# stevebottos/owl-vit-object-detection

Measured on AMD Instinct MI355X. Metric: train images/sec, OWL-ViT-B/16 768x768, higher is better.
Workload: dtype bf16; 1 GPU; owlvit-base-patch16 bf16, batch=32/GPU, 768x768, full train step (matcher+loss+backward+AdamW); global_batch=32, parallelism=dp1, encoder_streams=2, weights=init, optimizer_schedule=in-line, windows=1

## Files before the change

### include/owl_hip.h

```cpp
#ifndef OWL_HIP_H
#define OWL_HIP_H
#include <stdint.h>

#ifdef __cplusplus
extern "C" {
#endif

#define OWL_ABI_VERSION 8
const char* owl_last_error(void);
int owl_abi_version(void);

int owl_gemm_nt_bf16(void* stream, int epi, const void* A, int64_t lda, int64_t a_rows, const void* W, int64_t ldw, int64_t w_rows, const float* bias, void* out, int64_t ldo, const float* resid, void* aux, int64_t ld_aux, int64_t M, int64_t N, int64_t K, float alpha, int splits, int64_t Tp, int tile);
#define OWL_GEMM_KERNEL_SP128 0
#define OWL_GEMM_KERNEL_SP256 1
#define OWL_GEMM_KERNEL_PP2 2
#define OWL_GEMM_KERNEL_PPH 3
int owl_gemm_nt_plan(int epi, int64_t M, int64_t N, int64_t K, int64_t a_rows, int has_aux, int64_t Tp, int splits, int tile, int* kernels, int64_t* rows);
int owl_gemm_effective_splits(int64_t K, int splits);
int owl_gemm_slab_workspace_bytes(int64_t M, int64_t ldo, int64_t K, int splits, int64_t* bytes);
int owl_slab_reduce(void* stream, const float* slabs, float* out, int64_t n, int64_t slab_stride, int nsplit, int accumulate);

int owl_patch_embed_scratch_bytes(int64_t B, int64_t S, int64_t ps, int64_t D, int tile, int64_t* bytes);
int owl_patch_embed_bf16(void* stream, const void* image_bf16, const void* w_pe, const float* pos, float* x_out, void* scratch, int64_t B, int64_t S, int64_t ps, int64_t D, int64_t Tp, int tile);
int owl_cls_rows(void* stream, float* x, const float* cls, const float* pos, int64_t B, int64_t Tp, int64_t D);
// ... 41 lines not shown
int owl_preprocess_color_workspace_bytes(int64_t n_tiles, int64_t out_h, int64_t out_w, int64_t* bytes);
int owl_preprocess_u8_tiles_color(void* stream, const void* desc, const float* color, int64_t n_tiles, int64_t max_rows, unsigned char* tmp, void* workspace, int64_t workspace_bytes, const float* lut, void* out, int out_bf16, int64_t n_out, int64_t out_h, int64_t out_w);
int owl_normalize_u8(void* stream, const unsigned char* src, int src_chw, const float* lut, void* out, int out_bf16, int64_t n_images, int64_t H, int64_t W);

int owl_text_embed(void* stream, const int64_t* ids, const float* tok_emb, const float* pos_emb, float* x, int64_t N, int64_t S, int64_t W, int64_t vocab);
int owl_causal_attention_small(void* stream, const void* qkv_bf16, void* out_bf16, int64_t N, int64_t S, int64_t heads, float scale);
int owl_text_pool_project(void* stream, const float* x, const int64_t* ids, const float* gamma, const float* beta, const float* wproj, float* out, int64_t N, int64_t S, int64_t W, int64_t Pdim, float eps);

int owl_gemm_tn_slab_bf16(void* stream, const void* dY, int64_t ldy, const void* X, int64_t ldx, const void* zero_row, float* slab, int64_t M, int64_t N, int64_t K, int splits, int* splits_used, int variant, float* bias_slab);
int owl_colsum_bf16(void* stream, const void* in_bf16, int64_t ld, float* colsum, int64_t R, int64_t C, float* partials, int64_t partials_floats);
int owl_gemm_tn_slab_workspace_bytes(int64_t M, int64_t N, int64_t K, int splits, int64_t* bytes);

int owl_box_pairwise(void* stream, const float* boxes1, const float* boxes2, float* out3, int64_t N, int64_t M);

int owl_rowreduce_workspace_bytes(int64_t groups, int64_t rows_per_group, int64_t C, int64_t* bytes);
int owl_layernorm_bwd(void* stream, const void* dy, int dy_bf16, const float* x, const float* stats, const float* gamma, const float* dres, float* dx, float* dgamma, float* dbeta, int64_t rows, int64_t D, void* dx_bf16, float* partials, int64_t partials_floats, float* dx_colsum);
int owl_merge_ln_bwd(void* stream, const float* dfeats, const float* x, const float* cls_ln, const float* stats1, const float* stats2, const float* g1, const float* b1, const float* g2, float* dx, float* dcls_ws, float* dg1, float* db1, float* dg2, float* db2, int64_t B, int64_t P, int64_t Tp, int64_t D, float* partials, int64_t partials_floats, void* dx_bf16, float* dx_colsum);
int owl_class_sims_bwd(void* stream, const float* dsims, const float* sims, const unsigned char* argmax, const float* inv_norm, const float* e, const float* qhat32, void* de_bf16, void* g_bf16, void* e_bf16, int64_t rows, int64_t Dt, int64_t C);
int owl_query_normalize_bwd(void* stream, const float* dqhat, const float* queries, float* dqueries, int64_t nq, int64_t Dt);
int owl_class_sims_wide_bwd(void* stream, const float* dsims, const float* sims, const unsigned char* argmax, const float* inv_norm, const float* e, const float* qhat_wide, void* de_bf16, void* g_bf16, void* e_bf16, int64_t rows, int64_t Dt, int64_t C, int64_t Qp);
int owl_query_normalize_wide_bwd(void* stream, const float* dqhat_wide, const float* queries, float* dqueries, int64_t nq, int64_t Dt);
int owl_box_final_bwd_blocks(int64_t rows);
int owl_box_final_bwd(void* stream, const float* dboxes, const float* sig, const void* h1_bf16, const void* u1_bf16, const float* w2, void* du1_bf16, float* partials, float* dw2_db2, int64_t rows, int64_t D, float* du1_colsum);
int owl_transpose_colsum_bf16(void* stream, const void* in, int64_t ld_in, void* out_t, int64_t ld_out, float* colsum, int64_t R, int64_t C, float* partials, int64_t partials_floats);
int owl_colsum_f32(void* stream, const float* in, float* colsum, int64_t R, int64_t C, float* partials, int64_t partials_floats);
int owl_embed_bwd(void* stream, const float* dx, float* dpos, float* dcls, void* dE_bf16, int64_t B, int64_t T, int64_t Tp, int64_t D);
int owl_im2row_bf16(void* stream, const void* image_bf16, void* out_bf16, int64_t ld_out, int64_t B, int64_t S, int64_t ps);
int owl_slab_reduce_rows(void* stream, const float* slabs, float* out, int64_t rows, int64_t cols, int64_t ld_slab, int64_t slab_stride, int nsplit, int accumulate);

int owl_adamw_step(void* stream, float* p, const float* g, float* m, float* v, void* p_bf16, int64_t n, float lr, float beta1, float beta2, float eps, float weight_decay, int64_t step, float grad_scale);

int owl_grad_norm_workspace_bytes(int64_t n, int64_t* bytes);
int owl_grad_sumsq(void* stream, const float* g, int64_t n, void* workspace);
int owl_adamw_step_grouped(void* stream, float* p, const float* g, float* m, float* v, void* p_bf16, int64_t n, float lr, float beta1, float beta2, float eps, float weight_decay, int64_t step, float grad_scale, const int64_t* seg_end, const float* seg_lr, const float* seg_wd, int nseg, float max_norm, const void* workspace, float* norm_out);

int owl_ema_update(void* stream, float* ema, const float* p, int64_t n, float d, float w);
int owl_adamw_step_ema(void* stream, float* p, const float* g, float* m, float* v, void* p_bf16, int64_t n, float lr, float beta1, float beta2, float eps, float weight_decay, int64_t step, float grad_scale, const int64_t* seg_end, const float* seg_lr, const float* seg_wd, int nseg, float max_norm, const void* workspace, float* norm_out, float* ema, float d, float w);

int owl_prefix_emit(void* stream, const float* xs, const void* delta1_bf16, const void* delta2_bf16, int64_t n, int64_t block_elems, const int64_t* dst_addr, const int64_t* slot_addr);
int owl_prefix_gather(void* stream, int64_t n, int64_t block_elems, const int64_t* src_addr, const int64_t* dst_addr);

int owl_image_query_workspace_bytes(int64_t N, int64_t P, int64_t Dt, int64_t* nbytes);
int owl_image_query_select(void* stream, const float* e, const float* boxes, const float* qbox, int64_t N, int64_t P, int64_t Dt, void* workspace, int64_t workspace_bytes, int* best, float* query, int* info, float* v_out, double* mean_out, double* sim_out);
int owl_query_bank_fill(void* stream, const float* query, const int* row_ptr, const int* members, float* bank, int64_t N, int64_t nq, int64_t Dt);

int owl_class_logits_fwd(void* stream, const float* e, const float* queries, const void* feats_bf16, const float* w_shift, const float* b_shift, const float* w_scale, const float* b_scale, const unsigned char* mask, float* rowstats, float* logits, float* scores, int64_t B, int64_t P, int64_t Q, int64_t nbanks, int64_t nmasks, int64_t Dt, int64_t D);
// ... 23 lines not shown
```

### owl-vit-object-detection_amd/autograd.py

```python
from collections import namedtuple

import torch

from . import _lib, ops


DW_ITEMS = 256
TN_SMALL_N = True
FOLD_BIAS_COLSUM = True


def _grads_attached(model) -> bool:
    for n, off in model.flat_offsets.items():
        g = model._byname[n].grad
        if g is None or g.data_ptr() != model.flat_grad.data_ptr() + 4 * off:
            return False
    return True


def _attach_grads(model):
    if _grads_attached(model):
        return
    keep = {}
    for n in model.flat_offsets:
# ... 85 lines not shown
            if head["event"] is not None:
                main.wait_event(head["event"])
        else:
            backward_impl(model, B, d_boxes, None, None, logit_head=head)
        hg = (None,) * ctx.n_head
        if dhead is not None:
            hg = (dhead[:D], dhead[2 * D:2 * D + 1], dhead[D:2 * D], dhead[2 * D + 1:])
        return (None, None, dq, None) + (None,) * nflat + hg


def _bws(model, B):
    key = ("bwd", B)
    if key in model._ws:
        return model._ws[key]
    cfg, dev = model.cfg, model.device_
    D, I, Tp, P, Dt, H = cfg.hidden, cfg.mlp, cfg.tokens_padded, cfg.patches, cfg.text_dim, cfg.heads
    M, Mh = B * Tp, B * P
    Mp, Mhp = ops.pad_rows(M), ops.pad_rows(Mh)
    bf, f32 = torch.bfloat16, torch.float32
    z = ops.zeros_rows
    Qg = _routed_cols(model)
    sz = _dw_sizes(cfg, Qg, model._train_emb)
    ws = dict(
        de=z(Mh, Dt, bf, dev), dqhat=torch.zeros(Qg, Dt, device=dev), du1=z(Mh, D, bf, dev), du0=z(Mh, D, bf, dev),
        g32=z(Mh, Qg, bf, dev), e_bf=z(Mh, Dt, bf, dev),
        box_part=torch.zeros(_lib.load().owl_box_final_bwd_blocks(Mh), 5 * D + 4, device=dev),
        slab=torch.zeros(sz.slab, device=dev),
        sink=torch.zeros(4 * D + 8, device=dev),
        bslab=torch.zeros(256 * max(3 * D, I, Dt), device=dev), bslab2=torch.zeros(256 * max(D, Dt), device=dev),
        dfeats=z(Mh, D, f32, dev), dcls=torch.zeros(B, D, device=dev),
        dx=z(M, D, f32, dev), dxb=z(M, D, bf, dev), du=z(M, I, bf, dev), dh=z(M, D, bf, dev), dxm=z(M, D, f32, dev),
        datt=z(M, D, bf, dev), dqkv=z(M, 3 * D, bf, dev),
        dvec=torch.zeros(B, H, Tp, device=dev),
        part=ops.rowreduce_workspace(B, Tp, max(3 * D, I, Dt), dev),
        part2=ops.rowreduce_workspace(B, Tp, max(3 * D, I, Dt), dev),
        dxb2=z(M, D, bf, dev),
        tA=torch.zeros(sz.tok_rows, Mp, dtype=bf, device=dev) if sz.tok_rows else None,
        tB=torch.zeros(sz.tok_rows, Mp, dtype=bf, device=dev) if sz.tok_rows else None,
        tAh=torch.zeros(sz.tAh_rows, Mhp, dtype=bf, device=dev),
        tBh=torch.zeros(sz.tBh_rows, Mhp, dtype=bf, device=dev),
        wT=torch.zeros(max(3 * D, I) * max(D, I), dtype=bf, device=dev),
        slab2=torch.zeros(sz.slab2, device=dev),
        wT2=torch.zeros(Dt * D, dtype=bf, device=dev),
        tn_all=sz.tn_all,
    )
    ws["dw_main"] = dict(slab=ws["slab"], part=ws["part"], bslab=ws["bslab"], tA=ws["tAh"], tB=ws["tBh"], tn_all=sz.tn_all)
    ws["dw_class"] = dict(slab=ws["slab2"], part=ws["part2"], bslab=ws["bslab2"], tA=ws["tAh"], tB=ws["tBh"], tn_all=sz.tn_all)
    ws["dw_enc"] = dict(slab=ws["slab"], part=ws["part2"], bslab=ws["bslab"], tA=ws["tA"], tB=ws["tB"], tn_all=sz.tn_all)
    model._ws[key] = ws
    return ws


def _split_k(n_rows_out, n_cols_out, k):
    t = 256 if (n_rows_out >= 512 and n_cols_out >= 256) else 128
    tiles = ((n_rows_out + t - 1) // t) * ((n_cols_out + t - 1) // t)
    slots = 256 if t == 256 else 512
    return max(1, min(k // 64, slots // tiles))


def _qkv_grads(model, i):
    D, pre = model.cfg.hidden, f"backbone.encoder.layers.{i}.self_attn.q_proj."
    o, ob = model.flat_offsets[pre + "weight"], model.flat_offsets[pre + "bias"]
    return model.flat_grad[o: o + 3 * D * D].view(3 * D, D), model.flat_grad[ob: ob + 3 * D]


def _routed_cols(model):
    return ops.wide_qp(model.cfg.n_classes) if model.wide_head else 32


DwPlan = namedtuple("DwPlan", "tn splits n_in_pad slab_elems")
DwSizes = namedtuple("DwSizes", "tn_all slab slab2 tok_rows tAh_rows tBh_rows")


def _dw_plan(n_out, n_in, *, bias=False, tn_all=False, rows=None):
    if n_in % 256 == 0 and (n_out % 256 == 0 or (TN_SMALL_N and n_out % 8 == 0 and n_out <= 64 and tn_all and not bias)):
# ... 46 lines not shown
    if scratch is None:
        plan, ld, dev = _dw_plan(D, K), ops.pad_rows(rows), dE.device
        scratch = dict(slab=torch.zeros(plan.slab_elems, device=dev),
                       tA=None if plan.tn else torch.zeros(D, ld, dtype=torch.bfloat16, device=dev), tB=None if plan.tn else torch.zeros(K, ld, dtype=torch.bfloat16, device=dev))
    weight_grad(dE, patches, grad_w, D, K, rows, scratch, accumulate=accumulate)


def backward_impl(model, B, d_boxes, d_sims, sims, logit_head=None):
    cfg = model.cfg
    D, I, H, Tp, T, P, Dt, C = cfg.hidden, cfg.mlp, cfg.heads, cfg.tokens_padded, cfg.tokens, cfg.patches, cfg.text_dim, cfg.n_classes
    M, Mh = B * Tp, B * P
    ws, bw = model._workspace(B), _bws(model, B)
    P_ = model._byname
    model._wait_params()
    model._grad_clean = False
    _attach_grads(model)
    G = lambda n: P_[n].grad
    tv = model._tview
    units, tls, floor, low = model._units, model._tl_set, model.backward_floor, model._chain_low
    t_q, t_cls, t_box = "queries" in units, "class_predictor.dense0" in units, "box_head" in units
    below_heads = floor != "heads"
    below_enc = floor in ("pre_layernorm", "embeddings")
    LP = lambda i: f"backbone.encoder.layers.{i}."
    d_boxes = d_boxes.contiguous().float()
    if logit_head is None:
        d_sims = d_sims.contiguous().float()
    else:
        d_logits = logit_head["dlogits"].contiguous().float()

    pre_wt = model._wt if (getattr(model, "pretranspose", False) and model._wt_event is not None) else None
    if pre_wt is not None:
        torch.cuda.current_stream().wait_event(model._wt_event)

    def wT(name, rows, cols, buf=bw["wT"]):
        if name not in model.flat_offsets:
            return model._fz[name + ".T"]
        if pre_wt is not None:
            return pre_wt[name]
        out = buf[: rows * cols].view(cols, rows)
        ops.transpose_bf16(tv(name), out, rows, cols)
        return out

    S, J, fork = model._bwd_streams()
    main0 = torch.cuda.current_stream()
    hs = S(1) if (model.head_streams and model.encoder_streams > 1 and len(model._encoder_chunks(B)) > 1 and bw["tn_all"]) else main0
    ev_h = model._dw_events
# ... 21 lines not shown
                                     workspace=bw[key], **more)
                if t_cls:
                    weight_grad(bw["de"], ws["feats"], G("class_predictor.dense0.weight"), Dt, D, Mh, cdw, G("class_predictor.dense0.bias"))
                if below_heads:
                    ops.gemm(ops.EPI_ACC_F32, bw["de"], wT("class_predictor.dense0.weight", Dt, D, buf=cw), bw["dfeats"], M=Mh, N=D, K=Dt)
        elif t_q or t_cls or below_heads:
            if model.wide_head:
                Qp = bw["g32"].shape[1]
                ops.class_sims_wide_bwd(d_sims, sims, ws["argmax"], ws["inv_norm"], ws["e"], ws["qhat"], bw["de"], bw["g32"], bw["e_bf"], Mh, Dt, C)
                if t_q:
                    weight_grad(bw["g32"], bw["e_bf"], bw["dqhat"], Qp, Dt, Mh, cdw, accumulate=0)
                    ops.query_normalize_wide_bwd(bw["dqhat"], P_["queries"], G("queries"), cfg.queries, Dt)
            else:
                ops.class_sims_bwd(d_sims, sims, ws["argmax"], ws["inv_norm"], ws["e"], ws["qhat"], bw["de"], bw["g32"], bw["e_bf"], Mh, Dt, C)
                if t_q:
                    weight_grad(bw["g32"], bw["e_bf"], bw["dqhat"], 32, Dt, Mh, cdw, accumulate=0)
                    _lib.call("owl_query_normalize_bwd", ops.stream(), bw["dqhat"], P_["queries"], G("queries"), cfg.queries, Dt)
            if t_cls:
                weight_grad(bw["de"], ws["feats"], G("class_predictor.dense0.weight"), Dt, D, Mh, cdw, G("class_predictor.dense0.bias"))
            if below_heads:
                ops.gemm(ops.EPI_F32, bw["de"], wT("class_predictor.dense0.weight", Dt, D, buf=cw), bw["dfeats"], M=Mh, N=D, K=Dt)
        if hs is not main0:
            ev_h[1].record(hs)
    w0T = None
    if t_box or below_heads:
        if t_box:
            gw2, gb2 = G("box_head.dense2.weight"), G("box_head.dense2.bias")
            assert gb2.data_ptr() == gw2.data_ptr() + 4 * gw2.numel(), "dense2 weight/bias grads must be adjacent in the flat bucket"
        else:
            gw2 = bw["sink"]
        ops.box_final_bwd(d_boxes, ws["sig"], ws["hb1"], ws["ub1"], P_["box_head.dense2.weight"], bw["du1"], bw["box_part"], gw2, Mh, D,
                          du1_colsum=G("box_head.dense1.bias") if t_box else None)
        if t_box:
            weight_grad(bw["du1"], ws["hb0"], G("box_head.dense1.weight"), D, D, Mh, bw["dw_main"])
        ops.gemm(ops.EPI_DGELU_BF16, bw["du1"], wT("box_head.dense1.weight", D, D), bw["du0"], aux=ws["ub0"], M=Mh, N=D, K=D)
        if t_box:
            weight_grad(bw["du0"], ws["feats"], G("box_head.dense0.weight"), D, D, Mh, bw["dw_main"], G("box_head.dense0.bias"))
        if below_heads:
            w0T = wT("box_head.dense0.weight", D, D)
    if hs is not main0:
        main0.wait_event(ev_h[1])
    if logit_head is not None and logit_head.get("event") is not None:
        logit_head["event"].record(main0)
    if not below_heads:
        return
    ops.gemm(ops.EPI_ACC_F32, bw["du0"], w0T, bw["dfeats"], M=Mh, N=D, K=D)
    sink = bw["sink"]
    t_pl, t_ppl = "backbone.post_layernorm" in units, "post_post_layernorm" in units
    last = cfg.layers - 1
    ops.merge_ln_bwd(bw["dfeats"], ws["x_fin"], ws["cls_ln"], ws["st_post"], ws["st_pp"], P_["backbone.post_layernorm.weight"],
                     P_["backbone.post_layernorm.bias"], P_["post_post_layernorm.weight"], bw["dx"], bw["dcls"],
                     G("backbone.post_layernorm.weight") if t_pl else sink[:D], G("backbone.post_layernorm.bias") if t_pl else sink[D:2 * D],
                     G("post_post_layernorm.weight") if t_ppl else sink[2 * D:3 * D], G("post_post_layernorm.bias") if t_ppl else sink[3 * D:4 * D],
                     B, P, Tp, D, partials=bw["part"], dx_bf16=bw["dxb"],
                     dx_colsum=G(LP(last) + "mlp.fc2.bias") if last in tls else None)
    if low is None:
        return
    scale = cfg.head_dim ** -0.5

    def dx_only(layers):
        chunks = model._encoder_chunks(B)
        main = torch.cuda.current_stream()
        streams = [main] + [S(c) for c in range(1, len(chunks))]
        if len(chunks) > 1:
            fork.record(main)
            for s_ in streams[1:]:
                s_.wait_event(fork)
        for i in layers:
            Ls, fz = model._layer_ws(B, i), model._fz
# ... 101 lines not shown
```

### owl-vit-object-detection_amd/losses.py

```python
import torch
import torch.nn as nn

from . import _lib, ops
from .matcher import HungarianMatcher, PackedTargets, box_iou, generalized_box_iou
from .matcher import OpenVocabMatcher, _mask_u8, pack_open_vocab_targets


class _PushPullFn(torch.autograd.Function):
    @staticmethod
    def forward(ctx, pred_sims, pred_boxes, crit, tg):
        B, P, C = pred_sims.shape
        dev = pred_sims.device
        sims = pred_sims.detach().contiguous().float()
        boxes = pred_boxes.detach().contiguous().float()
        tc, pred_idx, tgt_idx, _ = crit.matcher.match_packed(sims, boxes, tg)
        s = ops.stream()
        _lib.call("owl_spread_labels", s, boxes, tc, B, P, crit.background_label, 0.85)
        need = pred_sims.requires_grad or pred_boxes.requires_grad
        per_image = torch.empty(B, 4, device=dev)
        losses = torch.empty(4, device=dev)
        dsims = torch.empty(B, P, C, device=dev) if need else None
        dl1 = torch.empty(B, P, 4, device=dev) if need else None
        dgiou = torch.empty(B, P, 4, device=dev) if need else None
        _lib.call("owl_push_pull_loss", s, sims, boxes, tc, crit.scales, tg.boxes, pred_idx, tgt_idx, tg.counts, per_image,
                  losses, dsims, dl1, dgiou, B, P, C, tg.Nmax, crit.background_label)
        ctx.saved = (tc, dsims, dl1, dgiou, B, P, C, crit.background_label)
        crit.last = dict(target_classes=tc, pred_idx=pred_idx, tgt_idx=tgt_idx, per_image=per_image, sizes=tg.sizes)
        return losses[0], losses[1], losses[2], losses[3]

    @staticmethod
    def backward(ctx, g0, g1, g2, g3):
        tc, dsims, dl1, dgiou, B, P, C, bg = ctx.saved
        dev = tc.device
        g = torch.stack([g0, g1, g2, g3]).to(device=dev, dtype=torch.float32)
        out_sims = torch.empty(B, P, C, device=dev)
        out_boxes = torch.empty(B, P, 4, device=dev)
        _lib.call("owl_push_pull_loss_bwd", ops.stream(), g, tc, dsims, dl1, dgiou, out_sims, out_boxes, B, P, C, bg)
        return out_sims, out_boxes, None, None


class PushPullLoss(nn.Module):
    def __init__(self, n_classes, scales):
        super().__init__()
        self.matcher = HungarianMatcher(n_classes)
        self.scales = None if scales is None else torch.as_tensor(scales, dtype=torch.float32)
        self.background_label = n_classes
        self.last = None

    def pack(self, target_classes, target_boxes, device):
        if isinstance(target_classes, PackedTargets):
            return target_classes
        labels = list(target_classes) if not torch.is_tensor(target_classes) else list(target_classes.unbind(0))
        boxes = list(target_boxes) if not torch.is_tensor(target_boxes) else list(target_boxes.unbind(0))
        return PackedTargets(labels, boxes, device, self.background_label)

    def forward(self, predicted_classes, target_classes, predicted_boxes, target_boxes=None):
        dev = predicted_classes.device
        if self.scales is not None and self.scales.device != dev:
            self.scales = self.scales.to(dev)
        tg = self.pack(target_classes, target_boxes, dev)
        if len(tg.sizes) != predicted_classes.shape[0]:
# ... 2 lines not shown
        return {"loss_ce": ce, "loss_bg": bg, "loss_bbox": l1, "loss_giou": giou}


class _OpenVocabFn(torch.autograd.Function):
    @staticmethod
    def forward(ctx, logits, pred_boxes, crit, tg, mask_u8, nmasks, num_boxes):
        B, P, Q = logits.shape
        dev = logits.device
        lg = logits.detach().contiguous().float()
        boxes = pred_boxes.detach().contiguous().float()
        tc, pred_idx, tgt_idx, _ = crit.matcher.match_packed(lg, boxes, tg, mask_u8, nmasks)
        s = ops.stream()
        need = logits.requires_grad or pred_boxes.requires_grad
        nbytes = torch.zeros(1, dtype=torch.int64)
        _lib.call("owl_focal_loss_workspace_bytes", B, P, Q, nbytes)
        ws = torch.empty(int(nbytes.item()) // 8, dtype=torch.float64, device=dev)
        losses = torch.empty(3, device=dev)
        dl1 = torch.empty(B, P, 4, device=dev) if need else None
        dgiou = torch.empty(B, P, 4, device=dev) if need else None
        _lib.call("owl_focal_loss_fwd", s, lg, mask_u8, tc, ws, ws.numel() * 8, B, P, Q, nmasks, float(crit.alpha))
        _lib.call("owl_box_pair_loss", s, boxes, mask_u8, tg.labels, tg.boxes, pred_idx, tgt_idx, tg.counts, ws, ws.numel() * 8, dl1, dgiou, B, P, Q, nmasks, tg.Nmax)
        _lib.call("owl_open_vocab_loss_reduce", s, ws, ws.numel() * 8, losses, B, P, Q, float(num_boxes))
        ctx.saved = (lg, mask_u8, nmasks, tc, dl1, dgiou, float(crit.alpha), float(num_boxes))
        crit.last = dict(target_classes=tc, pred_idx=pred_idx, tgt_idx=tgt_idx, sizes=tg.sizes, num_boxes=float(num_boxes))
        return losses[0], losses[1], losses[2]

    @staticmethod
    def backward(ctx, g0, g1, g2):
        lg, mask_u8, nmasks, tc, dl1, dgiou, alpha, num_boxes = ctx.saved
        B, P, Q = lg.shape
        dev = lg.device
        g = torch.stack([g0, g1, g2]).to(device=dev, dtype=torch.float32)
        dlogits = torch.empty(B, P, Q, device=dev)
        dboxes = torch.empty(B, P, 4, device=dev)
        s = ops.stream()
        _lib.call("owl_focal_loss_bwd", s, g, lg, mask_u8, tc, dlogits, B, P, Q, nmasks, alpha, num_boxes)
        _lib.call("owl_box_pair_loss_bwd", s, g, dl1, dgiou, dboxes, B, P, num_boxes)
        return dlogits, dboxes, None, None, None, None, None


class OpenVocabLoss(nn.Module):

    def __init__(self, alpha=0.25, class_cost=1, bbox_cost=5, giou_cost=2, gamma=2, box_format="xyxy"):
        super().__init__()
        if gamma != 2:
            raise ValueError("OpenVocabLoss: gamma is 2 (the kernels square the modulating factor); other values are not built")
        if box_format not in ("xyxy", "cxcywh"):
            raise ValueError(f"box_format must be 'xyxy' or 'cxcywh', got {box_format!r}")
        self.matcher = OpenVocabMatcher(class_cost, bbox_cost, giou_cost)
        self.alpha = float(alpha)
        self.box_format = box_format
        self.last = None

    def forward(self, logits, pred_boxes, targets, query_mask=None, num_boxes=None):
        if logits.dim() != 3 or pred_boxes.shape != logits.shape[:2] + (4,):
            raise ValueError("logits must be [B, P, Q] and pred_boxes [B, P, 4]")
        B, P, Q = logits.shape
        tg = pack_open_vocab_targets(targets, logits.device, Q, query_mask, self.box_format)
        if len(tg.sizes) != B:
            raise ValueError("batch size mismatch between predictions and targets")
        if tg.Nmax > P:
# ... 9 lines not shown
```

### owl-vit-object-detection_amd/models.py

```python
import math
from collections import OrderedDict

import numpy as np
import torch
import torch.nn as nn

from . import _lib, ops, weights as W
from .config import OwlConfig, check_image_size, get_config, table_grid
from .postprocess import PostProcess
from .prefix_cache import PrefixCache, _id_list


def box_bias_table(grid: int) -> torch.Tensor:
    coords = torch.arange(1, grid + 1, dtype=torch.float32)
    xx, yy = torch.meshgrid(coords, coords, indexing="xy")
    bc = torch.stack((xx, yy), dim=-1)
    bc[..., 0] /= grid
    bc[..., 1] /= grid
    bc = torch.clip(bc.view(-1, 2), 0.0, 1.0)
    coord_bias = torch.log(bc + 1e-4) - torch.log1p(-bc + 1e-4)
    size = torch.full_like(coord_bias, 1.0)
    size[..., 0] /= grid
    size[..., 1] /= grid
    size_bias = torch.log(size + 1e-4) - torch.log1p(-size + 1e-4)
# ... 128 lines not shown
        self.box_bias = box_bias_table(cfg.grid).to(self.device_)
        self._pos_used = None
        if cfg.native_grid != cfg.grid:
            self._pos_used = torch.zeros(cfg.tokens, D, dtype=torch.float32, device=self.device_)
            self._refresh_pos()
            self.register_load_state_dict_post_hook(lambda module, incompatible: module._refresh_pos())
        self._ws = {}
        self._gen = 0
        self._ws_lru = []
        self.max_cached_batch_sizes = 2
        self._saved = None
        self._bf16_current = False
        self._bf16_version = None
        self.encoder_streams = int(encoder_streams)
        self._streams, self._join, self._fork_ev, self._fork_ev_tail = [], {}, None, None
        self.head_streams = True
        self._dw_events_ = None
        self._param_event = None
        self._grad_clean = False
        self.overlap_tail = False
        self._tail_stream_ = None
        self.pretranspose = False
        self._wt, self._wt_stream_, self._wt_event = None, None, None
        self._trainable = frozenset(order)
        self.register_state_dict_pre_hook(lambda module, prefix, keep_vars: module._wait_params())
        self.prefix_cache = None
        self.register_load_state_dict_post_hook(lambda module, incompatible: module._invalidate_prefix())
        self.logit_head = None
        self._logit_head_flat = None

    def _attach(self, dotted: str, p: nn.Parameter):
        parts = dotted.split(".")
        node = self
        for part in parts[:-1]:
            if part not in node._modules:
                node.add_module(part, _Node())
            node = node._modules[part]
        node.register_parameter(parts[-1], p)

    def p(self, name: str) -> torch.Tensor:
        return self._byname[name]

    def _tview(self, name: str, dtype=torch.bfloat16):
        o = self.flat_offsets[name]
        n = self._byname[name].numel()
        src = self.flat_bf16 if dtype == torch.bfloat16 else self.flat_param
# ... 773 lines not shown
```

### owl-vit-object-detection_amd/ops.py

```python
import torch

from . import _lib

EPI_BIAS_BF16, EPI_QGELU_BF16, EPI_GELU_BF16, EPI_RESID_F32, EPI_F32, EPI_ATOMIC_F32 = 0, 1, 2, 3, 4, 5
EPI_TRANS_BF16, EPI_PATCH_F32, EPI_DQGELU_BF16, EPI_DGELU_BF16, EPI_ACC_F32, EPI_SLAB_F32 = 6, 7, 8, 9, 10, 11

ROW_PAD = 128
CHIP_CUS = 256
ATTN_VARIANT = 0
GEMM_TILE = 0


def stream() -> int:
    return torch.cuda.current_stream().cuda_stream


def pad_rows(n: int) -> int:
    return (n + ROW_PAD - 1) // ROW_PAD * ROW_PAD


def zeros_rows(rows: int, width: int, dtype, device) -> torch.Tensor:
    return torch.zeros(pad_rows(rows), width, dtype=dtype, device=device)


# ... 352 lines not shown

def class_sims_wide_bwd(dsims, sims, argmax, inv_norm, e, qhat_wide, de, g, e_bf16, rows, Dt, C):
    _chk(g, torch.bfloat16, "g"); _chk(de, torch.bfloat16, "de"); _chk(e_bf16, torch.bfloat16, "e_bf16")
    Qp = wide_qp(C)
    if g.shape[-1] != Qp or g.numel() < rows * Qp or de.numel() < rows * Dt or e_bf16.numel() < rows * Dt:
        raise ValueError(f"class_sims_wide_bwd: g must be [rows, {Qp}], de / e_bf16 [rows, Dt]")
    _lib.call("owl_class_sims_wide_bwd", stream(), dsims, sims, argmax, inv_norm, e, qhat_wide, de, g, e_bf16, rows, Dt, C, Qp)


def query_normalize_wide_bwd(dqhat_wide, queries, dqueries, nq, Dt):
    _chk(dqhat_wide, torch.float32, "dqhat_wide"); _chk(queries, torch.float32, "queries"); _chk(dqueries, torch.float32, "dqueries")
    if dqhat_wide.numel() < 32 * wide_blocks(nq // 3) * Dt:
        raise ValueError("query_normalize_wide_bwd: dqhat_wide must hold [ceil(C / 10) * 32, Dt] floats")
    _lib.call("owl_query_normalize_wide_bwd", stream(), dqhat_wide, queries, dqueries, nq, Dt)


def box_final_bwd(dboxes, sig, h1, u1, w2, du1, partials, dw2_db2, rows, D, du1_colsum=None):
    if partials.numel() < _lib.load().owl_box_final_bwd_blocks(int(rows)) * (5 * int(D) + 4):
        raise ValueError("box_final_bwd: partials must hold owl_box_final_bwd_blocks(rows) x (5 D + 4) floats")
    _chk(du1_colsum, torch.float32, "du1_colsum")
    _lib.call("owl_box_final_bwd", stream(), dboxes, sig, h1, u1, w2, du1, partials, dw2_db2, rows, D, du1_colsum)


def transpose_colsum(src, dst, colsum, R, C, ld_in=None, ld_out=None, partials=None):
    part = _part(partials, R, C, src.device) if colsum is not None else None
    _lib.call("owl_transpose_colsum_bf16", stream(), src, ld_in if ld_in is not None else src.shape[-1], dst,
              (ld_out if ld_out is not None else dst.shape[-1]) if dst is not None else 0, colsum, R, C,
              part, part.numel() if part is not None else 0)


def colsum_f32(src, colsum, R, C, partials=None):
    part = _part(partials, R, C, src.device)
    _lib.call("owl_colsum_f32", stream(), src, colsum, R, C, part, part.numel())


def embed_bwd(dx, dpos, dcls, dE, B, T, Tp, D):
    _chk(dx, torch.float32, "dx"); _chk(dpos, torch.float32, "dpos"); _chk(dcls, torch.float32, "dcls"); _chk(dE, torch.bfloat16, "dE")
    if dx.numel() < B * Tp * D or dpos.numel() < T * D or dcls.numel() < D or dE.numel() < B * (T - 1) * D:
        raise ValueError("embed_bwd: dx must hold [B, Tp, D], dpos [T, D], dcls [D], dE [B (T - 1), D]")
    _lib.call("owl_embed_bwd", stream(), dx, dpos, dcls, dE, B, T, Tp, D)


def pos_resample(pos, out, g0, g, D):
    _chk(pos, torch.float32, "pos"); _chk(out, torch.float32, "out")
    if pos.numel() < (g0 * g0 + 1) * D or out.numel() < (g * g + 1) * D:
        raise ValueError("pos_resample: pos must hold [g0 g0 + 1, D], out [g g + 1, D]")
# ... 176 lines not shown
```

Measured before the change: 1257 images/sec.

## Run box-head backward GEMMs only on rows with nonzero box gradients

Box-loss gradients are nonzero only for matched predictions, at most B*Nmax rows. The new path compacts those row indices on the GPU, gathers the matching du1 and pre-GELU rows, and runs the dense1 input-gradient GEMM and the dense0 input-gradient GEMM on a small padded row set. The dense0 contribution is then scatter-added into dfeats, which replaces two full Mh x D x D GEMMs. The dense0 weight gradient still runs over all rows, using a zero buffer with the compacted rows written in and cleared afterwards. In exchange it adds several small launches, extra workspace, and a loss-side tag that carries the row cap; if the cap overflows, the gathered rows are filled with NaN rather than the path falling back to the dense computation.

```diff
diff --git a/include/owl_hip.h b/include/owl_hip.h
--- a/include/owl_hip.h
+++ b/include/owl_hip.h
@@ -87,6 +87,11 @@
 int owl_query_normalize_wide_bwd(void* stream, const float* dqhat_wide, const float* queries, float* dqueries, int64_t nq, int64_t Dt);
 int owl_box_final_bwd_blocks(int64_t rows);
 int owl_box_final_bwd(void* stream, const float* dboxes, const float* sig, const void* h1_bf16, const void* u1_bf16, const float* w2, void* du1_bf16, float* partials, float* dw2_db2, int64_t rows, int64_t D, float* du1_colsum);
+int owl_box_rows_compact_blocks(int64_t rows);
+int owl_box_rows_compact(void* stream, const float* dboxes, int64_t rows, int64_t cap, int* row_list, int* count_flag);
+int owl_box_rows_put(void* stream, const void* src0, const void* src1, void* dst0, void* dst1, const int* row_list, const int* count_flag, int64_t rows, int64_t cap, int64_t D);
+int owl_box_rows_gather(void* stream, const void* src0, const void* src1, const void* src2, void* dst0, void* dst1, void* dst2, const int* row_list, const int* count_flag, int64_t rows, int64_t cap_pad, int64_t D);
+int owl_box_rows_scatter_add(void* stream, const float* dfc, float* dfeats, const int* row_list, const int* count_flag, int64_t rows, int64_t cap, int64_t D);
 int owl_transpose_colsum_bf16(void* stream, const void* in, int64_t ld_in, void* out_t, int64_t ld_out, float* colsum, int64_t R, int64_t C, float* partials, int64_t partials_floats);
 int owl_colsum_f32(void* stream, const float* in, float* colsum, int64_t R, int64_t C, float* partials, int64_t partials_floats);
 int owl_embed_bwd(void* stream, const float* dx, float* dpos, float* dcls, void* dE_bf16, int64_t B, int64_t T, int64_t Tp, int64_t D);
diff --git a/owl-vit-object-detection_amd/autograd.py b/owl-vit-object-detection_amd/autograd.py
--- a/owl-vit-object-detection_amd/autograd.py
+++ b/owl-vit-object-detection_amd/autograd.py
@@ -131,9 +131,8 @@
     Qg = _routed_cols(model)
     sz = _dw_sizes(cfg, Qg, model._train_emb)
     ws = dict(
-        de=z(Mh, Dt, bf, dev), dqhat=torch.zeros(Qg, Dt, device=dev), du1=z(Mh, D, bf, dev), du0=z(Mh, D, bf, dev),
+        de=z(Mh, Dt, bf, dev), dqhat=torch.zeros(Qg, Dt, device=dev),
         g32=z(Mh, Qg, bf, dev), e_bf=z(Mh, Dt, bf, dev),
-        box_part=torch.zeros(_lib.load().owl_box_final_bwd_blocks(Mh), 5 * D + 4, device=dev),
         slab=torch.zeros(sz.slab, device=dev),
         sink=torch.zeros(4 * D + 8, device=dev),
         bslab=torch.zeros(256 * max(3 * D, I, Dt), device=dev), bslab2=torch.zeros(256 * max(D, Dt), device=dev),
@@ -160,6 +159,50 @@
     return ws
 
 
+def _box_dense_ws(model, B, bw, du0=True):
+    D, Mh, dev = model.cfg.hidden, B * model.cfg.patches, model.device_
+    if "du1" not in bw:
+        bw["du1"] = ops.zeros_rows(Mh, D, torch.bfloat16, dev)
+        bw["box_part"] = torch.zeros(_lib.load().owl_box_final_bwd_blocks(Mh), 5 * D + 4, device=dev)
+    if du0 and "du0" not in bw:
+        bw["du0"] = ops.zeros_rows(Mh, D, torch.bfloat16, dev)
+    return bw
+
+
+def _box_rows_ws(model, B, bw, cap_pad):
+    rw = bw.get("box_rows")
+    if rw is None or rw["cap_pad"] < cap_pad:
+        D, dev = model.cfg.hidden, model.device_
+        bf, z = torch.bfloat16, ops.zeros_rows
+        rw = dict(cap_pad=cap_pad, row_list=torch.zeros(cap_pad, dtype=torch.int32, device=dev),
+                  count_flag=torch.zeros(ops.box_rows_state_ints(B * model.cfg.patches), dtype=torch.int32, device=dev),
+                  du1c=z(cap_pad, D, bf, dev), du0c=z(cap_pad, D, bf, dev), ub0c=z(cap_pad, D, bf, dev), dfc=z(cap_pad, D, torch.float32, dev),
+                  du0z=None if rw is None else rw["du0z"])
+        bw["box_rows"] = rw
+    if "box_head" in model._units and rw["du0z"] is None:
+        rw["du0z"] = ops.zeros_rows(B * model.cfg.patches, model.cfg.hidden, torch.bfloat16, model.device_)
+    return rw
+
+
+BOX_ROWS_MARK = "_owl_box_rows_cap"
+
+
+def mark_box_rows(d_boxes, cap):
+    setattr(d_boxes, BOX_ROWS_MARK, int(cap))
+    return d_boxes
+
+
+def _box_rows_cap(model, d_boxes, B, P):
+    cap = getattr(d_boxes, BOX_ROWS_MARK, None)
+    if cap is None or getattr(model, "box_backward", "auto") != "auto":
+        return None
+    if d_boxes.dtype != torch.float32 or not d_boxes.is_contiguous() or tuple(d_boxes.shape) != (B, P, 4):
+        return None
+    if ops.box_rows_cap_pad(cap) * 8 > B * P:
+        return None
+    return int(cap)
+
+
 def _split_k(n_rows_out, n_cols_out, k):
     t = 256 if (n_rows_out >= 512 and n_cols_out >= 256) else 128
     tiles = ((n_rows_out + t - 1) // t) * ((n_cols_out + t - 1) // t)
@@ -252,6 +295,9 @@
     below_heads = floor != "heads"
     below_enc = floor in ("pre_layernorm", "embeddings")
     LP = lambda i: f"backbone.encoder.layers.{i}."
+    if getattr(model, "box_backward", "auto") not in ("auto", "dense"):
+        raise ValueError(f"model.box_backward must be 'auto' or 'dense', got {model.box_backward!r}")
+    box_cap = _box_rows_cap(model, d_boxes, B, P)
     d_boxes = d_boxes.contiguous().float()
     if logit_head is None:
         d_sims = d_sims.contiguous().float()
@@ -319,8 +365,10 @@
                 ops.gemm(ops.EPI_F32, bw["de"], wT("class_predictor.dense0.weight", Dt, D, buf=cw), bw["dfeats"], M=Mh, N=D, K=Dt)
         if hs is not main0:
             ev_h[1].record(hs)
-    w0T = None
+    w0T = rw = None
     if t_box or below_heads:
+        model.last_box_backward = "dense" if box_cap is None else "rows"
+        _box_dense_ws(model, B, bw, du0=box_cap is None)
         if t_box:
             gw2, gb2 = G("box_head.dense2.weight"), G("box_head.dense2.bias")
             assert gb2.data_ptr() == gw2.data_ptr() + 4 * gw2.numel(), "dense2 weight/bias grads must be adjacent in the flat bucket"
@@ -330,18 +378,35 @@
                           du1_colsum=G("box_head.dense1.bias") if t_box else None)
         if t_box:
             weight_grad(bw["du1"], ws["hb0"], G("box_head.dense1.weight"), D, D, Mh, bw["dw_main"])
-        ops.gemm(ops.EPI_DGELU_BF16, bw["du1"], wT("box_head.dense1.weight", D, D), bw["du0"], aux=ws["ub0"], M=Mh, N=D, K=D)
-        if t_box:
-            weight_grad(bw["du0"], ws["feats"], G("box_head.dense0.weight"), D, D, Mh, bw["dw_main"], G("box_head.dense0.bias"))
-        if below_heads:
-            w0T = wT("box_head.dense0.weight", D, D)
+        if box_cap is not None:
+            cap_pad = ops.box_rows_cap_pad(box_cap)
+            rw = _box_rows_ws(model, B, bw, cap_pad)
+            rl, cf = rw["row_list"], rw["count_flag"]
+            ops.box_rows_compact(d_boxes, Mh, box_cap, rl, cf)
+            ops.box_rows_gather([(bw["du1"], rw["du1c"]), (ws["ub0"], rw["ub0c"])], rl, cf, Mh, cap_pad, D)
+            ops.gemm(ops.EPI_DGELU_BF16, rw["du1c"], wT("box_head.dense1.weight", D, D), rw["du0c"], aux=rw["ub0c"], M=cap_pad, N=D, K=D)
+            if t_box:
+                ops.box_rows_put([(rw["du0c"], rw["du0z"])], rl, cf, Mh, box_cap, D)
+                weight_grad(rw["du0z"], ws["feats"], G("box_head.dense0.weight"), D, D, Mh, bw["dw_main"], G("box_head.dense0.bias"))
+                ops.box_rows_put([(None, rw["du0z"])], rl, cf, Mh, box_cap, D)
+            if below_heads:
+                ops.gemm(ops.EPI_F32, rw["du0c"], wT("box_head.dense0.weight", D, D), rw["dfc"], M=cap_pad, N=D, K=D)
+        else:
+            ops.gemm(ops.EPI_DGELU_BF16, bw["du1"], wT("box_head.dense1.weight", D, D), bw["du0"], aux=ws["ub0"], M=Mh, N=D, K=D)
+            if t_box:
+                weight_grad(bw["du0"], ws["feats"], G("box_head.dense0.weight"), D, D, Mh, bw["dw_main"], G("box_head.dense0.bias"))
+            if below_heads:
+                w0T = wT("box_head.dense0.weight", D, D)
     if hs is not main0:
         main0.wait_event(ev_h[1])
     if logit_head is not None and logit_head.get("event") is not None:
         logit_head["event"].record(main0)
     if not below_heads:
         return
-    ops.gemm(ops.EPI_ACC_F32, bw["du0"], w0T, bw["dfeats"], M=Mh, N=D, K=D)
+    if rw is not None:
+        ops.box_rows_scatter_add(rw["dfc"], bw["dfeats"], rw["row_list"], rw["count_flag"], Mh, box_cap, D)
+    else:
+        ops.gemm(ops.EPI_ACC_F32, bw["du0"], w0T, bw["dfeats"], M=Mh, N=D, K=D)
     sink = bw["sink"]
     t_pl, t_ppl = "backbone.post_layernorm" in units, "post_post_layernorm" in units
     last = cfg.layers - 1
diff --git a/owl-vit-object-detection_amd/csrc/box_rows_bwd.hip b/owl-vit-object-detection_amd/csrc/box_rows_bwd.hip
--- /dev/null
+++ b/owl-vit-object-detection_amd/csrc/box_rows_bwd.hip
@@ -0,0 +1,154 @@
+#include "common.h"
+
+
+__device__ __forceinline__ bool box_row_nonzero(const float4& g) {
+    return !(g.x == 0.f) || !(g.y == 0.f) || !(g.z == 0.f) || !(g.w == 0.f);
+}
+
+#define BOX_ROWS_CB 1024
+
+__device__ __forceinline__ int box_rows_block_sum(int v, int* lds16) {
+    const int t = threadIdx.x;
+#pragma unroll
+    for (int o = 32; o > 0; o >>= 1) v += __shfl_xor(v, o, 64);
+    __syncthreads();
+    if ((t & 63) == 0) lds16[t >> 6] = v;
+    __syncthreads();
+    int s = 0;
+#pragma unroll
+    for (int w = 0; w < BOX_ROWS_CB / 64; w++) s += lds16[w];
+    return s;
+}
+
+__global__ __launch_bounds__(BOX_ROWS_CB) void box_rows_count_kernel(const float* __restrict__ dboxes, int64_t rows, int* __restrict__ block_count) {
+    __shared__ int lds16[BOX_ROWS_CB / 64];
+    const int64_t r = (int64_t)blockIdx.x * BOX_ROWS_CB + threadIdx.x;
+    const int nz = (r < rows && box_row_nonzero(*(const float4*)(dboxes + r * 4))) ? 1 : 0;
+    const int n = box_rows_block_sum(nz, lds16);
+    if (threadIdx.x == 0) block_count[blockIdx.x] = n;
+}
+
+__global__ __launch_bounds__(BOX_ROWS_CB) void box_rows_compact_kernel(const float* __restrict__ dboxes, int64_t rows, int cap, const int* __restrict__ block_count,
+                                                                       int* __restrict__ row_list, int* __restrict__ count_flag) {
+    __shared__ int lds16[BOX_ROWS_CB / 64];
+    __shared__ int wave_tot[BOX_ROWS_CB / 64];
+    const int t = threadIdx.x, lane = t & 63, wave = t >> 6;
+    int before = 0;
+    for (int j = t; j < (int)blockIdx.x; j += BOX_ROWS_CB) before += block_count[j];
+    const int base = box_rows_block_sum(before, lds16);
+    const int64_t r = (int64_t)blockIdx.x * BOX_ROWS_CB + t;
+    const bool nz = r < rows && box_row_nonzero(*(const float4*)(dboxes + r * 4));
+    const unsigned long long m = __ballot(nz);
+    if (lane == 0) wave_tot[wave] = __popcll(m);
+    __syncthreads();
+    int at = base + __popcll(m & ((1ull << lane) - 1ull)), own = 0;
+#pragma unroll
+    for (int w = 0; w < BOX_ROWS_CB / 64; w++) {
+        const int v = wave_tot[w];
+        if (w < wave) at += v;
+        own += v;
+    }
+    if (nz && at < cap) row_list[at] = (int)r;
+    if (blockIdx.x == gridDim.x - 1) {
+        const int total = base + own, count = min(total, cap);
+        for (int i = count + t; i < cap; i += BOX_ROWS_CB) row_list[i] = 0;
+        if (t == 0) { count_flag[0] = count; count_flag[1] = total > cap ? 1 : 0; }
+    }
+}
+
+struct BoxRowsPutP {
+    const uint4* src[2];
+    uint4* dst[2];
+};
+__global__ __launch_bounds__(128) void box_rows_put_kernel(BoxRowsPutP p, const int* __restrict__ row_list, const int* __restrict__ count_flag, int64_t rows, int D8) {
+    const uint4* src = p.src[blockIdx.y];
+    uint4* dst = p.dst[blockIdx.y];
+    const int i = blockIdx.x;
+    if (!dst || i >= count_flag[0]) return;
+    const int r = row_list[i];
+    if (r < 0 || r >= rows) return;
+    for (int c = threadIdx.x; c < D8; c += 128) dst[(int64_t)r * D8 + c] = src ? src[(int64_t)i * D8 + c] : make_uint4(0, 0, 0, 0);
+}
+
+struct BoxRowsGatherP {
+    const uint4* src[3];
+    uint4* dst[3];
+};
+__global__ __launch_bounds__(128) void box_rows_gather_kernel(BoxRowsGatherP p, const int* __restrict__ row_list, const int* __restrict__ count_flag,
+                                                              int64_t rows, int D8) {
+    const uint4* src = p.src[blockIdx.y];
+    uint4* dst = p.dst[blockIdx.y];
+    if (!src || !dst) return;
+    const int i = blockIdx.x;
+    int r = -1;
+    if (i < count_flag[0]) {
+        r = row_list[i];
+        if (r < 0 || r >= rows) r = -1;
+    }
+    const bool overflow = count_flag[1] != 0;
+    const uint4 qnan = make_uint4(0x7fc07fc0u, 0x7fc07fc0u, 0x7fc07fc0u, 0x7fc07fc0u);
+    for (int c = threadIdx.x; c < D8; c += 128)
+        dst[(int64_t)i * D8 + c] = r >= 0 ? (overflow ? qnan : src[(int64_t)r * D8 + c]) : make_uint4(0, 0, 0, 0);
+}
+
+__global__ __launch_bounds__(256) void box_rows_scatter_add_kernel(const float* __restrict__ dfc, float* __restrict__ dfeats, const int* __restrict__ row_list,
+                                                                   const int* __restrict__ count_flag, int64_t rows, int D4) {
+    const int i = blockIdx.x;
+    if (i >= count_flag[0]) return;
+    const int r = row_list[i];
+    if (r < 0 || r >= rows) return;
+    const float4* s = (const float4*)dfc + (int64_t)i * D4;
+    float4* d = (float4*)dfeats + (int64_t)r * D4;
+    for (int c = threadIdx.x; c < D4; c += 256) {
+        const float4 a = d[c], b = s[c];
+        d[c] = make_float4(a.x + b.x, a.y + b.y, a.z + b.z, a.w + b.w);
+    }
+}
+
+OWL_API int owl_box_rows_compact_blocks(int64_t rows) { return (int)((rows + BOX_ROWS_CB - 1) / BOX_ROWS_CB); }
+
+OWL_API int owl_box_rows_compact(void* stream, const float* dboxes, int64_t rows, int64_t cap, int* row_list, int* count_flag) {
+    OWL_CHECK_ARG(dboxes && row_list && count_flag, "owl_box_rows_compact: null pointer");
+    OWL_CHECK_ARG(rows >= 1 && rows < (1LL << 31) && cap >= 1 && cap < (1LL << 31), "owl_box_rows_compact: 1 <= rows, cap < 2^31");
+    const int nblk = owl_box_rows_compact_blocks(rows);
+    hipLaunchKernelGGL(box_rows_count_kernel, dim3((unsigned)nblk), dim3(BOX_ROWS_CB), 0, (hipStream_t)stream, dboxes, rows, count_flag + 2);
+    OWL_LAUNCH_CHECK();
+    hipLaunchKernelGGL(box_rows_compact_kernel, dim3((unsigned)nblk), dim3(BOX_ROWS_CB), 0, (hipStream_t)stream, dboxes, rows, (int)cap, (const int*)(count_flag + 2),
+                       row_list, count_flag);
+    OWL_LAUNCH_CHECK();
+    return 0;
+}
+
+OWL_API int owl_box_rows_put(void* stream, const void* src0, const void* src1, void* dst0, void* dst1, const int* row_list, const int* count_flag,
+                             int64_t rows, int64_t cap, int64_t D) {
+    OWL_CHECK_ARG(row_list && count_flag && (dst0 || dst1), "owl_box_rows_put: null pointer");
+    OWL_CHECK_ARG((!src0 || dst0) && (!src1 || dst1), "owl_box_rows_put: a source needs its destination");
+    OWL_CHECK_ARG(D >= 8 && D % 8 == 0 && rows >= 1 && rows < (1LL << 31) && cap >= 1 && cap < (1LL << 31), "owl_box_rows_put: D %% 8, 1 <= rows, cap < 2^31");
+    BoxRowsPutP p;
+    p.src[0] = (const uint4*)src0; p.src[1] = (const uint4*)src1; p.dst[0] = (uint4*)dst0; p.dst[1] = (uint4*)dst1;
+    hipLaunchKernelGGL(box_rows_put_kernel, dim3((unsigned)cap, 2), dim3(128), 0, (hipStream_t)stream, p, row_list, count_flag, rows, (int)(D / 8));
+    OWL_LAUNCH_CHECK();
+    return 0;
+}
+
+OWL_API int owl_box_rows_gather(void* stream, const void* src0, const void* src1, const void* src2, void* dst0, void* dst1, void* dst2,
+                                const int* row_list, const int* count_flag, int64_t rows, int64_t cap_pad, int64_t D) {
+    OWL_CHECK_ARG(row_list && count_flag, "owl_box_rows_gather: null pointer");
+    OWL_CHECK_ARG((!src0 == !dst0) && (!src1 == !dst1) && (!src2 == !dst2), "owl_box_rows_gather: a source and its destination go together");
+    OWL_CHECK_ARG(D >= 8 && D % 8 == 0 && rows >= 1 && rows < (1LL << 31) && cap_pad >= 1 && cap_pad < (1LL << 31), "owl_box_rows_gather: D %% 8, 1 <= rows, cap_pad < 2^31");
+    BoxRowsGatherP p;
+    p.src[0] = (const uint4*)src0; p.src[1] = (const uint4*)src1; p.src[2] = (const uint4*)src2;
+    p.dst[0] = (uint4*)dst0; p.dst[1] = (uint4*)dst1; p.dst[2] = (uint4*)dst2;
+    hipLaunchKernelGGL(box_rows_gather_kernel, dim3((unsigned)cap_pad, 3), dim3(128), 0, (hipStream_t)stream, p, row_list, count_flag, rows, (int)(D / 8));
+    OWL_LAUNCH_CHECK();
+    return 0;
+}
+
+OWL_API int owl_box_rows_scatter_add(void* stream, const float* dfc, float* dfeats, const int* row_list, const int* count_flag, int64_t rows,
+                                     int64_t cap, int64_t D) {
+    OWL_CHECK_ARG(dfc && dfeats && row_list && count_flag, "owl_box_rows_scatter_add: null pointer");
+    OWL_CHECK_ARG(D >= 4 && D % 4 == 0 && rows >= 1 && rows < (1LL << 31) && cap >= 1 && cap < (1LL << 31), "owl_box_rows_scatter_add: D %% 4, 1 <= rows, cap < 2^31");
+    hipLaunchKernelGGL(box_rows_scatter_add_kernel, dim3((unsigned)cap), dim3(256), 0, (hipStream_t)stream, dfc, dfeats, row_list, count_flag, rows, (int)(D / 4));
+    OWL_LAUNCH_CHECK();
+    return 0;
+}
diff --git a/owl-vit-object-detection_amd/losses.py b/owl-vit-object-detection_amd/losses.py
--- a/owl-vit-object-detection_amd/losses.py
+++ b/owl-vit-object-detection_amd/losses.py
@@ -2,6 +2,7 @@
 import torch.nn as nn
 
 from . import _lib, ops
+from .autograd import mark_box_rows
 from .matcher import HungarianMatcher, PackedTargets, box_iou, generalized_box_iou
 from .matcher import OpenVocabMatcher, _mask_u8, pack_open_vocab_targets
 
@@ -25,6 +26,7 @@
         _lib.call("owl_push_pull_loss", s, sims, boxes, tc, crit.scales, tg.boxes, pred_idx, tgt_idx, tg.counts, per_image,
                   losses, dsims, dl1, dgiou, B, P, C, tg.Nmax, crit.background_label)
         ctx.saved = (tc, dsims, dl1, dgiou, B, P, C, crit.background_label)
+        ctx.box_rows_cap = B * tg.Nmax
         crit.last = dict(target_classes=tc, pred_idx=pred_idx, tgt_idx=tgt_idx, per_image=per_image, sizes=tg.sizes)
         return losses[0], losses[1], losses[2], losses[3]
 
@@ -36,7 +38,7 @@
         out_sims = torch.empty(B, P, C, device=dev)
         out_boxes = torch.empty(B, P, 4, device=dev)
         _lib.call("owl_push_pull_loss_bwd", ops.stream(), g, tc, dsims, dl1, dgiou, out_sims, out_boxes, B, P, C, bg)
-        return out_sims, out_boxes, None, None
+        return out_sims, mark_box_rows(out_boxes, ctx.box_rows_cap), None, None
 
 
 class PushPullLoss(nn.Module):
@@ -85,6 +87,7 @@
         _lib.call("owl_box_pair_loss", s, boxes, mask_u8, tg.labels, tg.boxes, pred_idx, tgt_idx, tg.counts, ws, ws.numel() * 8, dl1, dgiou, B, P, Q, nmasks, tg.Nmax)
         _lib.call("owl_open_vocab_loss_reduce", s, ws, ws.numel() * 8, losses, B, P, Q, float(num_boxes))
         ctx.saved = (lg, mask_u8, nmasks, tc, dl1, dgiou, float(crit.alpha), float(num_boxes))
+        ctx.box_rows_cap = B * tg.Nmax
         crit.last = dict(target_classes=tc, pred_idx=pred_idx, tgt_idx=tgt_idx, sizes=tg.sizes, num_boxes=float(num_boxes))
         return losses[0], losses[1], losses[2]
 
@@ -99,7 +102,7 @@
         s = ops.stream()
         _lib.call("owl_focal_loss_bwd", s, g, lg, mask_u8, tc, dlogits, B, P, Q, nmasks, alpha, num_boxes)
         _lib.call("owl_box_pair_loss_bwd", s, g, dl1, dgiou, dboxes, B, P, num_boxes)
-        return dlogits, dboxes, None, None, None, None, None
+        return dlogits, mark_box_rows(dboxes, ctx.box_rows_cap), None, None, None, None, None
 
 
 class OpenVocabLoss(nn.Module):
diff --git a/owl-vit-object-detection_amd/models.py b/owl-vit-object-detection_amd/models.py
--- a/owl-vit-object-detection_amd/models.py
+++ b/owl-vit-object-detection_amd/models.py
@@ -174,6 +174,8 @@
         self._tail_stream_ = None
         self.pretranspose = False
         self._wt, self._wt_stream_, self._wt_event = None, None, None
+        self.box_backward = "auto"
+        self.last_box_backward = None
         self._trainable = frozenset(order)
         self.register_state_dict_pre_hook(lambda module, prefix, keep_vars: module._wait_params())
         self.prefix_cache = None
diff --git a/owl-vit-object-detection_amd/ops.py b/owl-vit-object-detection_amd/ops.py
--- a/owl-vit-object-detection_amd/ops.py
+++ b/owl-vit-object-detection_amd/ops.py
@@ -398,6 +398,57 @@
     _lib.call("owl_box_final_bwd", stream(), dboxes, sig, h1, u1, w2, du1, partials, dw2_db2, rows, D, du1_colsum)
 
 
+def box_rows_cap_pad(cap: int) -> int:
+    return (max(int(cap), 1) + 7) // 8 * 8
+
+
+def box_rows_state_ints(rows: int) -> int:
+    return 2 + _lib.load().owl_box_rows_compact_blocks(int(rows))
+
+
+def box_rows_compact(dboxes, rows, cap, row_list, count_flag):
+    _chk(dboxes, torch.float32, "dboxes"); _chk(row_list, torch.int32, "row_list"); _chk(count_flag, torch.int32, "count_flag")
+    rows, cap = int(rows), int(cap)
+    if dboxes.numel() < 4 * rows or row_list.numel() < cap or count_flag.numel() < box_rows_state_ints(rows):
+        raise ValueError("box_rows_compact: dboxes [rows, 4], row_list [>= cap], count_flag [box_rows_state_ints(rows)]")
+    _lib.call("owl_box_rows_compact", stream(), dboxes, rows, cap, row_list, count_flag)
+
+
+def box_rows_put(pairs, row_list, count_flag, rows, cap, D):
+    rows, cap, D = int(rows), int(cap), int(D)
+    if not 1 <= len(pairs) <= 2:
+        raise ValueError("box_rows_put: one or two (source, destination) pairs")
+    for src, dst in pairs:
+        _chk(src, torch.bfloat16, "src"); _chk(dst, torch.bfloat16, "dst")
+        if dst is None or dst.numel() < rows * D or dst.shape[-1] != D or (src is not None and (src.numel() < cap * D or src.shape[-1] != D)):
+            raise ValueError("box_rows_put: src [>= cap, D] or None, dst [>= rows, D]")
+    _chk(row_list, torch.int32, "row_list"); _chk(count_flag, torch.int32, "count_flag")
+    pairs = list(pairs) + [(None, None)] * (2 - len(pairs))
+    _lib.call("owl_box_rows_put", stream(), pairs[0][0], pairs[1][0], pairs[0][1], pairs[1][1], row_list, count_flag, rows, cap, D)
+
+
+def box_rows_gather(pairs, row_list, count_flag, rows, cap_pad, D):
+    pairs = [p for p in pairs if p is not None]
+    rows, cap_pad, D = int(rows), int(cap_pad), int(D)
+    if not 1 <= len(pairs) <= 3:
+        raise ValueError("box_rows_gather: one to three (source, destination) pairs")
+    for src, dst in pairs:
+        _chk(src, torch.bfloat16, "src"); _chk(dst, torch.bfloat16, "dst")
+        if src.numel() < rows * D or dst.numel() < cap_pad * D or src.shape[-1] != D or dst.shape[-1] != D:
+            raise ValueError("box_rows_gather: src [>= rows, D], dst [>= cap_pad, D]")
+    _chk(row_list, torch.int32, "row_list"); _chk(count_flag, torch.int32, "count_flag")
+    pairs = pairs + [(None, None)] * (3 - len(pairs))
+    _lib.call("owl_box_rows_gather", stream(), pairs[0][0], pairs[1][0], pairs[2][0], pairs[0][1], pairs[1][1], pairs[2][1], row_list, count_flag, rows, cap_pad, D)
+
+
+def box_rows_scatter_add(dfc, dfeats, row_list, count_flag, rows, cap, D):
+    _chk(dfc, torch.float32, "dfc"); _chk(dfeats, torch.float32, "dfeats"); _chk(row_list, torch.int32, "row_list"); _chk(count_flag, torch.int32, "count_flag")
+    rows, cap, D = int(rows), int(cap), int(D)
+    if dfc.numel() < cap * D or dfeats.numel() < rows * D:
+        raise ValueError("box_rows_scatter_add: dfc [>= cap, D], dfeats [>= rows, D]")
+    _lib.call("owl_box_rows_scatter_add", stream(), dfc, dfeats, row_list, count_flag, rows, cap, D)
+
+
 def transpose_colsum(src, dst, colsum, R, C, ld_in=None, ld_out=None, partials=None):
     part = _part(partials, R, C, src.device) if colsum is not None else None
     _lib.call("owl_transpose_colsum_bf16", stream(), src, ld_in if ld_in is not None else src.shape[-1], dst,
```

Measured after the change: 1272 images/sec, median of 6. 1.01x the previous value.
